# Jorgenlf/Drone-2d-custom-gym-env-for-reinforcement-learning

Measured on AMD Instinct MI355X. Metric: env-steps/sec at 65 536 parallel envs; 1/2/4/8 MI355X scaling, higher is better.
Workload: dtype f64

## Files before the change

### drone-2d-custom-gym-env-for-reinforcement-learning_amd/csrc/d2d_device.h

```cpp
#pragma once
#include <hip/hip_runtime.h>
#include <stdint.h>

#include "../../include/drone2d.h"
#include "d2d_pmath.h"

#pragma clang diagnostic ignored "-Wbitwise-instead-of-logical"

#ifdef D2D_BSTAMP
#define BST_N (1024 * 64 * 8)
__device__ uint64_t d2d_bst[BST_N];
#define BST_ARG , uint64_t* bst = nullptr
#define BST(k, dep)                                                                                      \
    do {                                                                                                 \
        if (bst) {                                                                                       \
            uint64_t bst_v;                                                                              \
            asm volatile("s_memtime %0\n\ts_waitcnt lgkmcnt(0)" : "=s"(bst_v) : "v"(dep));            \
            bst_t[k] = bst_v;                                                                            \
        }                                                                                                \
    } while (0)
#else
#define BST_ARG
#define BST(k, dep) \
    do {       \
// ... 305 lines not shown
constexpr double BR_GOLDEN = 0.3819660112501051;
constexpr double BR_XATOL3 = 1e-6 / 3.0;
constexpr int BT_K_MAX = 48;
template <class S>
__device__ __forceinline__ void brent_init(const S& s, const PathK& K, double px, double py, Brent& B) {
    B.a = 0.0 - 10.0;
    B.b = K.L + 10.0;
    B.fulc = B.a + BR_GOLDEN * (B.b - B.a);
    B.nfc = B.fulc;
    B.xf = B.fulc;
    B.rat = 0.0;
    B.e = 0.0;
    B.ia = u_index(s, B.a);
    B.ib = u_index(s, B.b);
    B.ka = SREC(s, REC_U1, B.ia);
    B.ixf = u_index(s, B.xf);
    B.fx = path_dist_n(s, K, B.xf, B.ixf, px, py, B.kxf);
    B.num = 1;
    B.ffulc = B.fx;
    B.fnfc = B.fx;
}
__device__ __forceinline__ bool brent_open(const Brent& B) {
    const double xm = 0.5 * (B.a + B.b);
    const double tol1 = BR_SQRT_EPS * fabs(B.xf) + BR_XATOL3;
    const double tol2 = 2.0 * tol1;
    return fabs(B.xf - xm) > (tol2 - 0.5 * (B.b - B.a));
}
__device__ __forceinline__ bool brent_active(const Brent& B) { return brent_open(B) & (B.num < 500); }
struct BrCand {
    double x;
    int ix;
};
template <bool KN, class S>
__device__ __forceinline__ int brent_interval(const S& s, const PathK& K, const Brent& B, double x, double ka,
                                              double* kn);
template <bool KN = false, class S>
__device__ __forceinline__ BrCand brent_cand(const S& s, const PathK& K, Brent& B, double* kn = nullptr) {
    const double a = B.a, b = B.b, xf = B.xf, fx = B.fx, nfc = B.nfc, fulc = B.fulc;
    const double ka = S::RM ? B.ka : SREC(s, REC_U1, B.ia);
    const double xm = 0.5 * (a + b);
    const double tol1 = BR_SQRT_EPS * fabs(xf) + BR_XATOL3;
    const double tol2 = 2.0 * tol1;
    const double r = (xf - nfc) * (fx - B.ffulc);
    double q = (xf - fulc) * (fx - B.fnfc);
    double p = (xf - fulc) * q - (xf - nfc) * r;
    q = 2.0 * (q - r);
    p = (q > 0.0) ? -p : p;
    q = fabs(q);
    const bool par = (fabs(B.e) > tol1) & (fabs(p) < fabs(0.5 * q * B.e)) & (p > q * (a - xf)) & (p < q * (b - xf));
    double rat_p = 0.0;
    if (__ballot(par) != 0ull) {
        rat_p = div_normal(p + 0.0, q);
        const double xp = xf + rat_p;
        const double d = xm - xf;
        rat_p = (((xp - a) < tol2) | ((b - xp) < tol2)) ? ((d < 0.0) ? -tol1 : tol1) : rat_p;
    }
    const double e_g = (xf >= xm) ? a - xf : b - xf;
    const double rat_g = BR_GOLDEN * e_g;
    B.e = par ? B.rat : e_g;
    const double rat = par ? rat_p : rat_g;
    B.rat = rat;
    const double mx = max_abs_fin(rat, tol1);
    const double x = xf + copysign(mx, rat);
    return BrCand{x, brent_interval<KN>(s, K, B, x, ka, kn)};
}
template <bool KN, class S>
__device__ __forceinline__ int brent_interval(const S& s, const PathK& K, const Brent& B, double x, double ka,
                                              double* kn) {
    const bool fast = B.ib <= B.ia + 1;
    int ix;
    if (__ballot(!fast) == 0ull) {
        ix = min(B.ia + ((x <= ka) ? 0 : 1), K.nw - 1);
    } else {
        if constexpr (S::RM) {
            int z = 0;
            asm volatile("" : "+v"(z));
            if constexpr (KN) {
                ix = u_index_kn(kn, K.nw, x, z);
            } else {
                ix = u_index_at(s, x, z);
            }
        } else {
            const S* sp = &s;
            asm volatile("" : "+v"(sp));
            ix = u_index(*sp, x);
        }
    }
    return ix;
}
template <class S>
__device__ __forceinline__ bool brent_update(Brent& B, const BrCand& c, double fu, double kx) {
    const double a = B.a, b = B.b, xf = B.xf, fx = B.fx, nfc = B.nfc, fulc = B.fulc;
    const double x = c.x;
    const int ix = c.ix;
    const bool le = fu <= fx;
    const bool c1 = !le & ((fu <= B.fnfc) | (nfc == xf));
    const bool c2 = !le & !c1 & ((fu <= B.ffulc) | (fulc == xf) | (fulc == nfc));
    const bool ge = x >= xf;
    const bool to_a = le == ge;
    const double t = le ? xf : x;
    const int ti = le ? B.ixf : ix;
    B.a = to_a ? t : a;
    B.b = to_a ? b : t;
    B.ia = to_a ? ti : B.ia;
    B.ib = to_a ? B.ib : ti;
    B.ixf = le ? ix : B.ixf;
    if constexpr (S::RM) {
        const double tk = le ? B.kxf : kx;
        B.ka = to_a ? tk : B.ka;
        B.kxf = le ? kx : B.kxf;
    }
    const double nfulc = (le | c1) ? nfc : (c2 ? x : fulc);
    const double nffulc = (le | c1) ? B.fnfc : (c2 ? fu : B.ffulc);
    const double nnfc = le ? xf : (c1 ? x : nfc);
    const double nfnfc = le ? fx : (c1 ? fu : B.fnfc);
    B.fulc = nfulc;
    B.ffulc = nffulc;
    B.nfc = nnfc;
    B.fnfc = nfnfc;
    B.xf = le ? x : xf;
    B.fx = min_fin(fu, fx);
    return le;
}
template <bool KN = false, class S>
__device__ __forceinline__ void brent_step(const S& s, const PathK& K, double px, double py, Brent& B,
                                           double* kn = nullptr BST_ARG) {
#ifdef D2D_BSTAMP
    uint64_t bst_t[5];
#endif
    BST(0, B.xf);
    const bool fast = B.ib <= B.ia + 1;
    const BrCand c = brent_cand<KN>(s, K, B, kn);
    BST(1, c.x);
    BST(2, c.ix);
    double kx;
    const double fu = path_dist_n(s, K, c.x, c.ix, px, py, kx);
    BST(3, fu);
    brent_update<S>(B, c, fu, kx);
#ifdef D2D_BSTAMP
    BST(4, B.fx);
    const uint64_t act = __ballot(1);
    if (bst && (int)(threadIdx.x & 63) == __ffsll((unsigned long long)act) - 1) {
        for (int k = 0; k < 5; ++k) bst[k] = bst_t[k];
        bst[5] = 0;
        bst[6] = (uint64_t)(__ballot(!fast) != 0ull);
        bst[7] = (uint64_t)__popcll(act);
    }
#else
    (void)fast;
#endif
}
template <bool KN = false, class S>
__device__ __forceinline__ void brent_run(const S& s, const PathK& K, double px, double py, Brent& B,
                                          double* kn = nullptr) {
    constexpr int IT_FREE = 500 - (BT_K_MAX + 1);
    for (int it = 0;; ++it) {
        bool act = brent_open(B);
        if (__builtin_expect(it >= IT_FREE, 0)) {
            asm volatile("" ::: "memory");
            act = act & (B.num + it < 500);
        }
        if (!act) break;
#ifdef D2D_BSTAMP
        uint64_t* bst = nullptr;
        if ((threadIdx.x >> 6) == 2 && blockIdx.x < 1024 && it < 64) bst = d2d_bst + ((size_t)blockIdx.x * 64 + it) * 8;
        brent_step<KN>(s, K, px, py, B, kn, bst);
#else
        brent_step<KN>(s, K, px, py, B, kn);
#endif
    }
}
template <bool KN = false, class S>
__device__ __forceinline__ double closest_u(const S& s, double px, double py, int& iu, double* kn = nullptr) {
    static_assert(!KN || S::RM, "staged knots / record cache: global-memory tables only");
    const PathK K = path_k(s);
    if constexpr (KN) {
#pragma unroll
        for (int k = 0; k < D2D_MAX_WPS; ++k) kn[64 * k + (threadIdx.x & 63)] = SUS(s, k);
    }
    Brent B;
    brent_init(s, K, px, py, B);
    brent_run<KN>(s, K, px, py, B, kn);
    iu = B.ixf;
    return B.xf;
}

constexpr int BT_K = BT_K_MAX;
constexpr int BT_HOT = BT_K + 3;
struct BtIt {
    double X, Y;
    double dxn, dxf;
    double e;
    double am, bm;
    double pad;
};
struct BtSnap {
    double a, b, fulc, nfc, xf, rat, e, ka, kxf;
    int32_t num, ia, ib, ixf;
    int32_t j_fulc, j_nfc, j_xf, pad;
};
struct BtHot {
    BtIt it[2][BT_HOT];
};
static_assert(sizeof(BtIt) == 64, "BtIt size");
struct BrTab {
    BtHot hot;
    BtSnap snap[2][BT_K + 1];
    int32_t len[2];
    int32_t pad[2];
};

template <class SC>
__device__ __forceinline__ void brtab_build(const SC& s, int kind, BrTab& T) {
    const PathK K = path_k(s);
    Brent B;
    B.a = 0.0 - 10.0;
    B.b = K.L + 10.0;
    B.fulc = B.a + BR_GOLDEN * (B.b - B.a);
    B.nfc = B.fulc;
    B.xf = B.fulc;
    B.rat = 0.0;
    B.e = 0.0;
    B.ia = u_index(s, B.a);
    B.ib = u_index(s, B.b);
    B.ka = SREC(s, REC_U1, B.ia);
    B.ixf = u_index(s, B.xf);
    B.num = 1;
    B.fx = B.ffulc = B.fnfc = 0.0;
    BtIt& h0 = T.hot.it[kind][0];
    path_eval_n(s, K, B.xf, B.ixf, h0.X, h0.Y, B.kxf);
    h0.dxn = h0.dxf = h0.e = h0.am = h0.bm = h0.pad = 0.0;
    int jf = 0, jn = 0, jx = 0;
    int k = 0;
    for (; k < BT_K && brent_active(B); ++k) {
        BtSnap& S = T.snap[kind][k];
        S = BtSnap{B.a, B.b, B.fulc, B.nfc, B.xf, B.rat, B.e, B.ka, B.kxf, B.num, B.ia, B.ib, B.ixf, jf, jn, jx, 0};
        const double a = B.a, b = B.b, xf = B.xf, nfc = B.nfc, fulc = B.fulc;
        const double xm = 0.5 * (a + b);
        const double tol1 = BR_SQRT_EPS * fabs(xf) + BR_XATOL3;
        BtIt& h = T.hot.it[kind][k + 1];
        h.dxn = xf - nfc;
        h.dxf = xf - fulc;
        h.e = (fabs(B.e) > tol1) ? B.e : 0.0;
        h.am = a - xf;
        h.bm = b - xf;
        h.pad = 0.0;
        const double e_g = (xf >= xm) ? a - xf : b - xf;
        const double rat = BR_GOLDEN * e_g;
        B.e = e_g;
        B.rat = rat;
        const double mx = max_abs_fin(rat, tol1);
        const double x = xf + ((rat < 0.0) ? -mx : mx);
        const int ix = u_index(s, x);
        double kx;
        path_eval_n(s, K, x, ix, h.X, h.Y, kx);
        B.num += 1;
        const bool le = !(kind == 0 && k == 0);
        const bool c1 = !le;
        const bool ge = x >= xf;
        const bool to_a = le == ge;
        const double t = le ? xf : x;
        const int ti = le ? B.ixf : ix;
        const double tk = le ? B.kxf : kx;
        B.a = to_a ? t : a;
        B.b = to_a ? b : t;
        B.ia = to_a ? ti : B.ia;
        B.ka = to_a ? tk : B.ka;
        B.ib = to_a ? B.ib : ti;
        B.ixf = le ? ix : B.ixf;
        B.kxf = le ? kx : B.kxf;
        const int j = k + 1;
        const double nfulc = (le | c1) ? nfc : fulc;
        const int njf = (le | c1) ? jn : jf;
        const double nnfc = le ? xf : (c1 ? x : nfc);
        const int njn = le ? jx : (c1 ? j : jn);
        B.fulc = nfulc;
        B.nfc = nnfc;
        B.xf = le ? x : xf;
        jf = njf;
        jn = njn;
        jx = le ? j : jx;
    }
    T.snap[kind][k] = BtSnap{B.a, B.b, B.fulc, B.nfc, B.xf, B.rat, B.e, B.ka, B.kxf, B.num, B.ia, B.ib, B.ixf,
                             jf, jn, jx, 0};
    T.len[kind] = k;
}

__device__ __forceinline__ double bt_check(const BtIt& h, int k, double px, double py, double ffulc, double fnfc,
                                           double fx, int& dev) {
    const double fu = norm2(h.X - px, h.Y - py);
    const double r = h.dxn * (fx - ffulc);
    double q = h.dxf * (fx - fnfc);
    double p = h.dxf * q - h.dxn * r;
    q = 2.0 * (q - r);
    p = (q > 0.0) ? -p : p;
    q = fabs(q);
    const bool par = (fabs(p) < fabs(0.5 * q * h.e)) & (p > q * h.am) & (p < q * h.bm);
    const bool ok = !par & (fu <= fx);
    dev = min(dev, ok ? BT_HOT : k);
    return fu;
}

template <bool LT>
__device__ __forceinline__ BtIt bt_hot(const BtHot* hot, int kind, int j) {
    if (!LT) return hot->it[kind][j];
    using HL = __attribute__((address_space(3))) const double;
    const HL* q = (const HL*)&hot->it[kind][j];
    return BtIt{q[0], q[1], q[2], q[3], q[4], q[5], q[6], q[7]};
}
template <bool LT>
__device__ __forceinline__ double bt_dist(const BtHot* hot, int kind, int j, double px, double py) {
    const BtIt h = bt_hot<LT>(hot, kind, j);
    return norm2(h.X - px, h.Y - py);
}
struct BtLane {
    int kind, len, dev;
    double fa, fb, fc;
};
template <bool LT>
__device__ __forceinline__ BtLane bt_start(const BrTab& T, const BtHot* hot, double px, double py) {
    const double f0 = bt_dist<LT>(hot, 0, 0, px, py);
    const double f1 = bt_dist<LT>(hot, 0, 1, px, py);
    BtLane L;
    L.kind = (f1 <= f0) ? 1 : 0;
    L.len = T.len[L.kind];
    L.dev = L.len;
    L.fa = f0;
    L.fb = L.kind ? f0 : f1;
    L.fc = L.kind ? f1 : f0;
    return L;
}
template <bool LT>
__device__ __forceinline__ void bt_window(const BtHot* hot, BtLane& L, int k, double px, double py) {
    L.fa = bt_dist<LT>(hot, L.kind, k - 2, px, py);
    L.fb = bt_dist<LT>(hot, L.kind, k - 1, px, py);
    L.fc = bt_dist<LT>(hot, L.kind, k, px, py);
}
template <bool LT>
__device__ __forceinline__ void bt_verify(const BtHot* hot, BtLane& L, int k0, int k1, double px, double py) {
    double fa = L.fa, fb = L.fb, fc = L.fc;
    int dev = L.dev;
    const int kind = L.kind;
    for (int k = k0; __ballot(k < min(dev, k1)) != 0ull; k += 3) {
        BtIt ha{}, hb{}, hc{};
        if (LT || k < min(dev, k1)) {
            ha = bt_hot<LT>(hot, kind, k + 1);
            hb = bt_hot<LT>(hot, kind, k + 2);
            hc = bt_hot<LT>(hot, kind, k + 3);
        }
        const double fd = bt_check(ha, k, px, py, fa, fb, fc, dev);
        const double fe = bt_check(hb, k + 1, px, py, fb, fc, fd, dev);
        const double ff = bt_check(hc, k + 2, px, py, fc, fd, fe, dev);
        fa = fd;
        fb = fe;
        fc = ff;
    }
    L.dev = min(dev, L.len);
    L.fa = fa;
    L.fb = fb;
    L.fc = fc;
}
template <bool LT, class SC>
__device__ __forceinline__ double bt_finish(const SC& s, const BrTab& T, const BtHot* hot, int kind, int dev,
                                            double px, double py, int& iu) {
    const BtSnap& S = T.snap[kind][dev];
    Brent B;
    B.a = S.a;
    B.b = S.b;
    B.fulc = S.fulc;
    B.nfc = S.nfc;
    B.xf = S.xf;
    B.rat = S.rat;
    B.e = S.e;
    B.ka = S.ka;
    B.kxf = S.kxf;
    B.num = S.num;
    B.ia = S.ia;
    B.ib = S.ib;
    B.ixf = S.ixf;
    if (__ballot(brent_active(B)) != 0ull) {
        const PathK K = path_k(s);
        B.ffulc = bt_dist<LT>(hot, kind, S.j_fulc, px, py);
        B.fnfc = bt_dist<LT>(hot, kind, S.j_nfc, px, py);
        B.fx = bt_dist<LT>(hot, kind, S.j_xf, px, py);
        brent_run(s, K, px, py, B);
    }
    iu = B.ixf;
    return B.xf;
}
template <bool LT, class S>
__device__ __forceinline__ double closest_u_tab(const S& s, const BrTab& T, const BtHot* hot, double px,
                                                double py, int& iu) {
    BtLane L = bt_start<LT>(T, hot, px, py);
    bt_verify<LT>(hot, L, 1, BT_K, px, py);
    return bt_finish<LT>(s, T, hot, L.kind, L.dev, px, py, iu);
}
__device__ __forceinline__ int bt_split(const BrTab& T) { return max(4, (T.len[0] + 3) / 2); }
__device__ __forceinline__ int bt_third(const BrTab& T, int p) {
    const int third = (T.len[0] + 2) / 3;
    return p == 0 ? 1 : (p >= 3 ? BT_K : 1 + p * third);
}
template <bool LT>
__device__ __forceinline__ void bt_window_snap(const BrTab& T, const BtHot* hot, BtLane& L, int k0, double px,
                                               double py) {
    const BtSnap& W = T.snap[L.kind][k0];
    L.fa = bt_dist<LT>(hot, L.kind, W.j_fulc, px, py);
    L.fb = bt_dist<LT>(hot, L.kind, W.j_nfc, px, py);
    L.fc = bt_dist<LT>(hot, L.kind, W.j_xf, px, py);
}

struct Body {
    double px, py, a, vx, vy, w;
};

constexpr double M_F = 0.2, M_M = 0.4;

__host__ __device__ constexpr double moment_box(double m, double w, double h) {
    double hw = w / 2.0, hh = h / 2.0;
    double vx[4] = {hw, hw, -hw, -hw}, vy[4] = {-hh, hh, hh, -hh};
    double s1 = 0.0, s2 = 0.0;
    for (int i = 0; i < 4; ++i) {
        double v1x = vx[i] + 0.0, v1y = vy[i] + 0.0;
        double v2x = vx[(i + 1) % 4] + 0.0, v2y = vy[(i + 1) % 4] + 0.0;
        double aa = v2x * v1y - v2y * v1x;
        double bb = (v1x * v1x + v1y * v1y) + (v1x * v2x + v1y * v2y) + (v2x * v2x + v2y * v2y);
        s1 += aa * bb;
        s2 += aa;
    }
    return (m * s1) / (6.0 * s2);
}
constexpr double MI_F = 1.0 / M_F, MI_M = 1.0 / M_M;
constexpr double II_F = 1.0 / moment_box(M_F, 100.0, 10.0);
constexpr double II_M = 1.0 / moment_box(M_M, 20.0, 20.0);

struct Arms {
    double m7c[2], m7s[2];
    double f47c, f47s, f40c, f40s, f33c, f33s;
};
__device__ __forceinline__ void arm(const Arms& A, int k, double& r1x, double& r1y, double& r2x, double& r2y) {
    const int m = k < 3 ? 0 : 1;
    const int q = k % 3;
    r1x = (q == 0) ? -A.m7c[m] : ((q == 1) ? 0.0 : A.m7c[m]);
    r1y = (q == 0) ? -A.m7s[m] : ((q == 1) ? 0.0 : A.m7s[m]);
    const double c = (k == 0 || k == 5) ? A.f47c : ((k == 1 || k == 4) ? A.f40c : A.f33c);
    const double s = (k == 0 || k == 5) ? A.f47s : ((k == 1 || k == 4) ? A.f40s : A.f33s);
    r2x = (k < 3) ? -c : c;
    r2y = (k < 3) ? -s : s;
}

constexpr int ARMS_N = 10;
__device__ __forceinline__ void arms_store(const Arms& A, double* ab, int stride) {
    const double v[ARMS_N] = {A.m7c[0], A.m7c[1], A.m7s[0], A.m7s[1], A.f47c, A.f47s,
                              A.f40c, A.f40s, A.f33c, A.f33s};
#pragma unroll
    for (int q = 0; q < 10; ++q) ab[q * stride] = v[q];
}
__device__ __forceinline__ void arm_lds(const double* ab, int stride, int k, double& r1x, double& r1y, double& r2x,
                                        double& r2y) {
    using LdsD = __attribute__((address_space(3))) double;
    const volatile LdsD* v = (const volatile LdsD*)ab;
    const int m = k < 3 ? 0 : 1;
    const int q = k % 3;
    const double mc = (q == 1) ? 0.0 : v[(0 + m) * stride], ms = (q == 1) ? 0.0 : v[(2 + m) * stride];
    r1x = (q == 0) ? -mc : ((q == 1) ? 0.0 : mc);
    r1y = (q == 0) ? -ms : ((q == 1) ? 0.0 : ms);
    const int f = (k == 0 || k == 5) ? 4 : ((k == 1 || k == 4) ? 6 : 8);
    const double c = v[f * stride], sn = v[(f + 1) * stride];
    r2x = (k < 3) ? -c : c;
    r2y = (k < 3) ? -sn : sn;
}

__device__ __forceinline__ void advance_position(Body& b) {
    b.px = fma(b.vx + 0.0, DT, b.px);
    b.py = fma(b.vy + 0.0, DT, b.py);
    b.a = fma(b.w + 0.0, DT, b.a);
}
template <class S>
__device__ __forceinline__ bool frame_hits(const S& s, const Body& F, double cs, double sn) {
    bool hit = false;
    for (int k = 0; k < s.n_circles; ++k) {
        const double dx = s.cx[k] - F.px, dy = s.cy[k] - F.py;
        {
            const double reach = s.cr[k] + 51.25;
            const bool near = (fabs(dx) < reach) & (fabs(dy) < reach);
            if (__ballot(near) == 0ull) continue;
        }
        const double lx = dx * cs + dy * sn;
        const double ly = -dx * sn + dy * cs;
        const double ex = lx - fmin(fmax(lx, -FRAME_HX), FRAME_HX), ey = ly - fmin(fmax(ly, -FRAME_HY), FRAME_HY);
        const double r = s.cr[k];
        hit |= (ex * ex + ey * ey <= r * r);
    }
    return hit;
}
template <class S>
__device__ __forceinline__ bool phys_positions(const S& s, Body B[3], double fL, double fR, double cs[3],
                                               double sn[3], double& fx, double& fy, double& tq) {
    double c0, s0;
    sincos_d(B[0].a, s0, c0);
    {
        const double tx = B[0].px - (0.0 * c0 - 0.0 * s0), ty = B[0].py - (0.0 * s0 + 0.0 * c0);
        const double cgx = c0 * 0.0 + (-s0) * 0.0 + tx, cgy = s0 * 0.0 + c0 * 0.0 + ty;
        double fwx = c0 * 0.0 + (-s0) * fL, fwy = s0 * 0.0 + c0 * fL;
        double rx = (c0 * -DRONE_R + (-s0) * 0.0 + tx) - cgx, ry = (s0 * -DRONE_R + c0 * 0.0 + ty) - cgy;
        fx = 0.0 + fwx;
        fy = 0.0 + fwy;
        tq = 0.0 + (rx * fwy - ry * fwx);
        fwx = c0 * 0.0 + (-s0) * fR;
        fwy = s0 * 0.0 + c0 * fR;
        rx = (c0 * DRONE_R + (-s0) * 0.0 + tx) - cgx;
        ry = (s0 * DRONE_R + c0 * 0.0 + ty) - cgy;
        fx = fx + fwx;
        fy = fy + fwy;
        tq += rx * fwy - ry * fwx;
    }
#pragma unroll
    for (int i = 0; i < 3; ++i) advance_position(B[i]);
    sincos_d(B[0].a, sn[0], cs[0]);
#pragma unroll
    for (int i = 1; i < 3; ++i) {
        const double d = B[i].a - B[0].a;
        if (!D2D_EXACT_TRIG && fabs(d) < 1e-2) {
            const double d2 = d * d;
            const double sd = d * fma(d2, fma(d2, fma(d2, -1.0 / 5040.0, 1.0 / 120.0), -1.0 / 6.0), 1.0);
            const double cdm1 = d2 * fma(d2, fma(d2, fma(d2, 1.0 / 40320.0, -1.0 / 720.0), 1.0 / 24.0), -0.5);
            sn[i] = fma(sn[0], cdm1, fma(cs[0], sd, sn[0]));
            cs[i] = fma(cs[0], cdm1, fma(-sn[0], sd, cs[0]));
        } else {
            sincos_d(B[i].a, sn[i], cs[i]);
        }
    }
    return frame_hits(s, B[0], cs[0], sn[0]);
}
template <class S>
__device__ __forceinline__ bool frame_advance(const S& s, Body& F) {
    advance_position(F);
    double sn, cs;
    sincos_d(F.a, sn, cs);
    return frame_hits(s, F, cs, sn);
}

__device__ __forceinline__ Arms make_arms(const double cs[3], const double sn[3]) {
    Arms A;
    A.m7c[0] = cs[1] * 7.0; A.m7s[0] = sn[1] * 7.0;
    A.m7c[1] = cs[2] * 7.0; A.m7s[1] = sn[2] * 7.0;
    A.f47c = cs[0] * 47.0; A.f47s = sn[0] * 47.0;
    A.f40c = cs[0] * 40.0; A.f40s = sn[0] * 40.0;
    A.f33c = cs[0] * 33.0; A.f33s = sn[0] * 33.0;
    return A;
}
// ... 385 lines not shown
```

### drone-2d-custom-gym-env-for-reinforcement-learning_amd/csrc/d2d_kernels.h

```cpp
#pragma once
#include <type_traits>

#include "d2d_curriculum.h"
#include "d2d_device.h"
#include "d2d_layout.h"

namespace d2dk {
using namespace d2d;

constexpr int BLOCK = 256;
constexpr int K1_THREADS = 256;
constexpr size_t K1_LDS_BUDGET = 40 * 1024;
constexpr size_t K2_LDS_BUDGET = 64 * 1024;
constexpr int PRIO_W0 = 2, PRIO_W1 = 1, PRIO_W2 = 3, PRIO_W3 = 1, PRIO_W2_POST = 0;

struct StepArgs {
    int n;
    int ns;
    int n_scn;
    double* st;
    int32_t* ist;
    double* acc;
    const void* scn;
    const BrTab* brt;
// ... 40 lines not shown
#define STAMP(k)                                                                                       \
    do {                                                                                               \
        if (a.stamps && (threadIdx.x & 63) == 0)                                                       \
            a.stamps[(size_t)(blockIdx.x * (blockDim.x >> 6) + (threadIdx.x >> 6)) * 8 + (k)] = __builtin_amdgcn_s_memtime(); \
        if (a.stamps && (threadIdx.x & 63) == 0 && (k) == 0)                                           \
            a.stamps[(size_t)(blockIdx.x * (blockDim.x >> 6) + (threadIdx.x >> 6)) * 8 + 7] =                          \
                ((uint64_t)__builtin_amdgcn_s_getreg((3 << 11) | 20) << 32) |                          \
                (uint32_t)__builtin_amdgcn_s_getreg((31 << 11) | 4) | ((uint64_t)(wave & 3) << 36) |   \
                ((uint64_t)(uint32_t)(wg + 1) << 40);                                                  \
    } while (0)
#define D2D_FSTAMP_BASE 65536
#define FSTAMP(k)                                                                                      \
    do {                                                                                               \
        if (a.stamps && (threadIdx.x & 63) == 0)                                                       \
            a.stamps[D2D_FSTAMP_BASE + (size_t)(blockIdx.x * (blockDim.x >> 6) + (threadIdx.x >> 6)) * 8 + (k)] =      \
                __builtin_amdgcn_s_memtime();                                                          \
    } while (0)
#else
#define STAMP(k) \
    do {         \
    } while (0)
#define FSTAMP(k) \
    do {          \
    } while (0)
#endif

__device__ __forceinline__ const BrTab* brtab(const StepArgs& a, int si) { return a.brt ? a.brt + si : nullptr; }
__device__ __forceinline__ size_t rc_entry(const StepArgs& a, int i, uint32_t ep) {
    return (size_t)(ep & 1u) * (size_t)a.ns + (size_t)i;
}

template <bool LDS, int NT, class S>
__device__ __forceinline__ const S* stage_scenarios(const StepArgs& a, S* lds, int first = 0, int count = -1) {
    if (!LDS) return scn_tab<S>(a);
    if (count < 0) count = a.n_scn;
    const int words = count * (int)(sizeof(S) / 8);
    const double* src = reinterpret_cast<const double*>(scn_tab<S>(a) + first);
    double* dst = reinterpret_cast<double*>(lds);
    for (int k = threadIdx.x; k < words; k += NT) dst[k] = src[k];
    return lds - first;
}
template <int NT>
__device__ __forceinline__ const BtHot* stage_hot(const StepArgs& a, BtHot* lds, int first = 0, int count = -1) {
    if (count < 0) count = a.n_scn;
    const int per = (int)(sizeof(BtHot) / 16);
    for (int k = threadIdx.x; k < count * per; k += NT) {
        const double2* src = reinterpret_cast<const double2*>(&a.brt[first + k / per].hot) + (k % per);
        reinterpret_cast<double2*>(lds)[k] = *src;
    }
    return lds - first;
}
template <int NWAVES>
__device__ __forceinline__ void glds_copy(void* lds_dst, const void* gsrc, int bytes) {
    using LP = __attribute__((address_space(3))) void;
    using GP = __attribute__((address_space(1))) void;
    const int wave = __builtin_amdgcn_readfirstlane(threadIdx.x >> 6), lane = threadIdx.x & 63;
    for (int c = wave; c * 1024 < bytes; c += NWAVES) {
        const int off = c * 1024 + lane * 16;
        if (off < bytes)
            __builtin_amdgcn_global_load_lds((GP*)((const char*)gsrc + off), (LP*)((char*)lds_dst + c * 1024), 16, 0, 0);
    }
}

__device__ __forceinline__ size_t fidx(int f, int n, int i) { return (size_t)f * (size_t)n + (size_t)i; }
template <typename T>
__device__ __forceinline__ T& fld(T* base, int f, int n, int i) {
    T* fb = base + (size_t)__builtin_amdgcn_readfirstlane(f) * (size_t)__builtin_amdgcn_readfirstlane(n);
    return fb[i];
}

__device__ __forceinline__ Body load_frame(const StepArgs& a, int i) {
    const int n = a.ns;
    return Body{fld(a.st, 0, n, i), fld(a.st, 1, n, i), fld(a.st, 2, n, i),
                fld(a.st, 3, n, i), fld(a.st, 4, n, i), fld(a.st, 5, n, i)};
}
template <class SC>
__device__ __forceinline__ void spawn_state(const StepArgs& a, const SC& S, int i, uint32_t ep, double sp[7]) {
    double x, y, th;
    spawn_draw(S, a.seed, (uint32_t)a.cfg.env_id_base + (uint32_t)i, ep, x, y, th);
    double sl, cl, sr, cr;
    sincos_d(th + PI, sl, cl);
    sincos_d(th, sr, cr);
    sp[0] = x;
    sp[1] = y;
    sp[2] = th;
    sp[3] = cl * DRONE_R + x;
    sp[4] = sl * DRONE_R + y;
    sp[5] = cr * DRONE_R + x;
    sp[6] = sr * DRONE_R + y;
}

using LdsU32 = __attribute__((address_space(3))) uint32_t;
__device__ __forceinline__ bool flag_seen(const uint32_t& f) {
    return __builtin_amdgcn_readfirstlane(*(const volatile LdsU32*)&f) != 0u;
}
__device__ __forceinline__ int pool_scenario(const StepArgs& a, int j, uint32_t ep) {
    return *a.pool_base + (a.pool_n > 1 ? pool_pick(a.seed, (uint32_t)a.cfg.env_id_base + (uint32_t)j, ep, a.pool_n) : 0);
}
__device__ __forceinline__ int fresh_slot(int j, uint32_t ep) { return 2 * j + (int)(ep & 1u); }
enum { FR_HEAD = 0, FR_TAIL0 = 1, FR_TAIL1 = 2, FR_WORDS = 4 };
__device__ __forceinline__ int next_scenario(const StepArgs& a, int j, uint32_t ep) {
    if (a.cfg.scn_pool == 2) return fresh_slot(j, ep);
    if (a.cfg.scn_pool) return pool_scenario(a, j, ep);
    if (a.n_scn <= 1) return 0;
    return a.env_scn[j];
}

struct K1Shared {
    double cas[6][EPB];
    int scn[EPB];
    uint8_t cause[EPB];
    uint8_t cvalid[EPB];
    uint32_t pflags[EPB];
    uint32_t ep[EPB];
    double sina[EPB];
    uint32_t w0t[EPB], w0fl[EPB];
    uint32_t f_done, f_ca, f_gs, f_rp, f_ver, f_ver1, f_acc, n_tile;
    double pe[2][EPB];
    double acc[D2D_NSTATS][EPB];
    union {
        struct {
            double jb[6 * JB_PER_JOINT][EPB];
            double arms[ARMS_N][EPB];
        } g;
        struct {
            double post[7][EPB];
            alignas(16) float obs[EPB * D2D_OBS_DIM];
        } p;
    } u;
};

__device__ __forceinline__ int lane_fresh() {
    int l;
    asm volatile("v_mbcnt_lo_u32_b32 %0, -1, 0\n\tv_mbcnt_hi_u32_b32 %0, -1, %0" : "=v"(l));
    return l;
}
__device__ __forceinline__ void flag_raise(uint32_t& f) {
    __builtin_amdgcn_fence(__ATOMIC_RELEASE, "workgroup");
    if ((threadIdx.x & 63) == 0) *(volatile LdsU32*)&f = 1u;
}
__device__ __forceinline__ void flag_wait(const uint32_t& f) {
    while (!flag_seen(f)) __builtin_amdgcn_s_sleep(1)  ;
    __builtin_amdgcn_fence(__ATOMIC_ACQUIRE, "workgroup");
}
__device__ __forceinline__ void tile_arrive(uint32_t& c) {
    __builtin_amdgcn_fence(__ATOMIC_RELEASE, "workgroup");
    if ((threadIdx.x & 63) == 0) atomicAdd(&c, 1u);
}
__device__ __forceinline__ void tile_wait(const uint32_t& c, uint32_t n) {
    while (__builtin_amdgcn_readfirstlane(*(const volatile LdsU32*)&c) < n) __builtin_amdgcn_s_sleep(1);
    __builtin_amdgcn_fence(__ATOMIC_ACQUIRE, "workgroup");
}

template <bool LDS, bool LTAB, bool GRP, class S>
__device__ __forceinline__ void k1_stage(const StepArgs& a, S* s_scn, int wg, const S*& scns,
                                         const BtHot*& hots, int& s0) {
    const int ws = (GRP && LDS) ? a.wg_scn[wg] : 0;
    s0 = ws >= 0 ? ws : -ws - 2;
    const int ncopy = (GRP && LDS) ? (ws >= 0 ? 1 : 2) : a.n_scn;
    hots = nullptr;
    if (LDS && (ncopy == 1 || !LTAB)) {
        glds_copy<K1_THREADS / 64>(s_scn, scn_tab<S>(a) + s0, (int)sizeof(S) * ncopy);
        if (LTAB) glds_copy<K1_THREADS / 64>(s_scn + 1, &a.brt[s0].hot, (int)sizeof(BtHot));
        scns = s_scn - s0;
        if (LTAB) hots = reinterpret_cast<const BtHot*>(s_scn + 1) - s0;
    } else {
        scns = stage_scenarios<LDS, K1_THREADS>(a, s_scn, s0, ncopy);
        if (LTAB) hots = stage_hot<K1_THREADS>(a, reinterpret_cast<BtHot*>(s_scn + ncopy), s0, ncopy);
    }
}

extern __shared__ __attribute__((aligned(16))) uint4 d2d_dyn_lds[];
constexpr int K1_KN_BYTES = D2D_MAX_WPS * 64 * 8;
template <bool LDS, bool LTAB, bool GRP, bool S3, class SC>
__device__ __forceinline__ void k1_body(const StepArgs& a, const SC* scns, const BtHot* hots, int s0, K1Shared& sh,
                                        int wg, int role, int qt) {
    const int wave = role;
    const int lane = threadIdx.x & 63;
    const bool gvalid = wg >= 0;
    const int e0 = gvalid ? wg * EPB : 0;
    const int i = e0 + lane;
    const int ie = (GRP && gvalid) ? a.lane_env[i] : i;
    const bool valid = gvalid && (GRP ? ie >= 0 : i < a.n);
    const int n = a.ns;
    const bool auto_reset = a.cfg.auto_reset != 0;
    STAMP(0);
    if (wg == 0 && qt == 0 && a.fill_ctl)
        __hip_atomic_store(&a.fill_ctl[0], __hip_atomic_load(&a.fill_ctl[1], __ATOMIC_RELAXED, __HIP_MEMORY_SCOPE_AGENT),
                           __ATOMIC_RELAXED, __HIP_MEMORY_SCOPE_AGENT);
    if (wg == 0 && qt == 0 && a.clock)
        __hip_atomic_fetch_add(a.clock, (int64_t)1, __ATOMIC_RELAXED, __HIP_MEMORY_SCOPE_AGENT);
    if (wave == 0) sh.scn[lane] = (valid && a.env_scn && a.n_scn > 1) ? a.env_scn[ie] : s0;
    if (S3 && wave == 0) sh.pflags[lane] = 0x7fffffffu;
    Body PF{};
    if (valid && wave != 0) PF = load_frame(a, i);
    if (qt == 0) {
        sh.f_done = 0u;
        sh.f_ca = 0u;
        sh.f_gs = 0u;
        sh.f_rp = 0u;
        sh.f_ver = 0u;
        sh.f_ver1 = 0u;
        sh.f_acc = 0u;
        sh.n_tile = 0u;
    }
    __syncthreads();
    STAMP(1);
    const SC& S = scns[sh.scn[lane]];
    float* const trow = a.tobs ? a.tobs + (size_t)ie * D2D_OBS_DIM : nullptr;
    float* const orow = &sh.u.p.obs[lane * D2D_OBS_DIM];

    Body F0{};
    double path_err = 0.0, tot_rew = 0.0;
    int t = 0, cause = 0;
    uint32_t flags = 0;
    RewardVel RV{};
    double dclose = 0.0, rew_sum = 0.0, rew_pp = 0.0, pdist = 0.0;
    uint32_t plal = 0;
    bool done = false;
    if (wave == 0) {
        __builtin_amdgcn_s_setprio(PRIO_W0);
        double ov[19];
        Body B[3];
        double j[12], cs[3], sn[3], fx = 0.0, fy = 0.0, tq = 0.0;
        if (valid) {
#pragma unroll
            for (int b = 0; b < 3; ++b) {
                B[b].px = fld(a.st, 6 * b + 0, n, i);
                B[b].py = fld(a.st, 6 * b + 1, n, i);
                B[b].a = fld(a.st, 6 * b + 2, n, i);
                B[b].vx = fld(a.st, 6 * b + 3, n, i);
                B[b].vy = fld(a.st, 6 * b + 4, n, i);
                B[b].w = fld(a.st, 6 * b + 5, n, i);
            }
#pragma unroll
            for (int k = 0; k < 12; ++k) j[k] = fld(a.st, D2D_S_J + k, n, i);
            t = fld(a.ist, D2D_I_T, n, i);
            flags = (uint32_t)fld(a.ist, D2D_I_FLAGS, n, i);
            const float2 act = reinterpret_cast<const float2*>(a.act)[ie];
            const float fs = (float)a.cfg.force_scale;
            const float lf = __fmul_rn(__fadd_rn(act.x / 2.0f, 0.5f), fs);
            const float rf = __fmul_rn(__fadd_rn(act.y / 2.0f, 0.5f), fs);
            if (phys_positions(S, B, (double)lf, (double)rf, cs, sn, fx, fy, tq)) flags |= D2D_FLAG_COLLIDED;
            t += 1;
            cause = end_cause(a.cfg, S, B[0], (flags & D2D_FLAG_COLLIDED) != 0, t);
            done = cause != 0;
            const int32_t ep = fld(a.ist, D2D_I_EPISODE, n, i);
            const bool cv = done && auto_reset && a.rc_tag[rc_entry(a, i, (uint32_t)ep)] == ep;
            sh.ep[lane] = (uint32_t)ep;
            sh.cause[lane] = (uint8_t)cause;
            sh.sina[lane] = sn[0];
            sh.cvalid[lane] = cv ? 1u : 0u;
            sh.w0t[lane] = (uint32_t)t;
            sh.w0fl[lane] = flags;
            if (!(done && auto_reset)) {
#pragma unroll
                for (int b = 0; b < 3; ++b) {
                    fld(a.st, 6 * b + 0, n, i) = B[b].px;
                    fld(a.st, 6 * b + 1, n, i) = B[b].py;
                    fld(a.st, 6 * b + 2, n, i) = B[b].a;
                }
            }
        }
        flag_raise(sh.f_done);
        if (valid) {
            const Arms A = make_arms(cs, sn);
            const double pos[6] = {B[0].px, B[0].py, B[1].px, B[1].py, B[2].px, B[2].py};
            double vel[9] = {B[0].vx, B[0].vy, B[0].w, B[1].vx, B[1].vy, B[1].w, B[2].vx, B[2].vy, B[2].w};
            phys_velocities<true>(A, pos, a.damping_dt, fx, fy, tq, vel, j, &sh.u.g.jb[0][lane], EPB,
                                  &sh.u.g.arms[0][lane]);
            asm volatile("" ::: "memory");
            const int ln = lane_fresh(), iw = e0 + ln;
            const uint32_t cw = sh.cause[ln];
            cause = (int)cw;
            done = cw != 0u;
            t = (int)sh.w0t[ln];
            flags = sh.w0fl[ln];
            if (!(done && auto_reset)) {
#pragma unroll
            for (int b = 0; b < 3; ++b) {
                fld(a.st, 6 * b + 3, n, iw) = vel[3 * b + 0];
                fld(a.st, 6 * b + 4, n, iw) = vel[3 * b + 1];
                fld(a.st, 6 * b + 5, n, iw) = vel[3 * b + 2];
            }
#pragma unroll
            for (int k = 0; k < 12; ++k) fld(a.st, D2D_S_J + k, n, iw) = j[k];
            }
            F0 = Body{0.0, 0.0, B[0].a, vel[0], vel[1], vel[2]};
        }
        flag_raise(sh.f_gs);
        STAMP(4);
        const int ln = lane_fresh(), iw = e0 + ln, iew = GRP ? ie : iw;
        const bool vw = gvalid && (GRP ? iew >= 0 : iw < a.n);
        if (vw) {
            float* const orw = &sh.u.p.obs[ln * D2D_OBS_DIM];
            float* const trw = a.tobs ? a.tobs + (size_t)iew * D2D_OBS_DIM : nullptr;
            sensor_vel(F0, sh.sina[ln], cs[0], ov);
            if (!(done && auto_reset)) {
                orw[0] = (float)ov[0];
                orw[1] = (float)ov[1];
                orw[2] = (float)ov[2];
                orw[17] = (float)ov[17];
                orw[18] = (float)ov[18];
            }
            if (done && trw) {
                trw[0] = (float)ov[0];
                trw[1] = (float)ov[1];
                trw[2] = (float)ov[2];
                trw[17] = (float)ov[17];
                trw[18] = (float)ov[18];
            }
        }
        tile_arrive(sh.n_tile);
        flag_wait(sh.f_ca);
        STAMP(5);
        if (vw) {
            CAStatic C;
            C.d = sh.cas[0][ln];
            C.os = sh.cas[1][ln];
            C.oc = sh.cas[2][ln];
            C.lpa = sh.cas[3][ln];
            C.lca = sh.cas[4][ln];
            C.rr = sh.cas[5][ln];
            RV = reward_vel(a.cfg, ov, C);
            dclose = C.d;
        }
        if (!S3) {
            flag_wait(sh.f_acc);
            const int lp = lane_fresh();
            path_err = sh.pe[0][lp];
            tot_rew = sh.pe[1][lp];
        }
        flag_wait(sh.f_rp);
        if (vw) {
            RewardPos RP{};
            RP.aa = sh.u.p.post[4][ln];
            RP.coll = sh.u.p.post[5][ln];
            RP.reach = sh.u.p.post[6][ln];
            RewardPath RQ{};
            RQ.ls = sh.u.p.post[0][ln];
            RQ.lc = sh.u.p.post[1][ln];
            RQ.pa = sh.u.p.post[2][ln];
            if (!GRP) {
                pdist = sh.u.p.post[3][ln];
                plal = sh.pflags[ln];
            }
            const RewardSum Q = reward_sum(a.cfg, RP, RV, RQ);
            rew_sum = Q.reward;
            rew_pp = Q.pp;
        }
    } else if (wave == 1) {
        float row[19];
        bool need = false;
        if (S3) {
            __builtin_amdgcn_s_setprio(PRIO_W2);
            if (valid && a.brt) {
                const BrTab& T = a.brt[sh.scn[lane]];
                const BtHot* hot = LTAB ? hots + sh.scn[lane] : &T.hot;
                Body F = PF;
                advance_position(F);
                BtLane L = bt_start<LTAB>(T, hot, F.px, F.py);
                const int k0 = bt_third(T, 1), k1 = bt_third(T, 2);
                if (k0 < min(k1, L.len)) {
                    if (k0 >= 4) bt_window<LTAB>(hot, L, k0, F.px, F.py);
                else bt_window_snap<LTAB>(T, hot, L, k0, F.px, F.py);
                    bt_verify<LTAB>(hot, L, k0, k1, F.px, F.py);
                }
                atomicMin(&sh.pflags[lane], (uint32_t)L.dev);
            }
            flag_raise(sh.f_ver1);
        }
        __builtin_amdgcn_s_setprio(PRIO_W1);
        if (valid) {
            Body F = PF;
            advance_position(F);
            double so[19];
            sensor_pos(a.cfg, S, F.px, F.py, F.a, so);
            const CAStatic C = ca_static(a.cfg, S, so);
            sh.cas[0][lane] = C.d;
            sh.cas[1][lane] = C.os;
            sh.cas[2][lane] = C.oc;
            sh.cas[3][lane] = C.lpa;
            sh.cas[4][lane] = C.lca;
            sh.cas[5][lane] = C.rr;
#pragma unroll
            for (int k = 0; k < 19; ++k) row[k] = (float)so[k];
        }
        flag_raise(sh.f_ca);
        flag_wait(sh.f_done);
        if (valid) {
            done = sh.cause[lane] != 0u;
            need = done && auto_reset;
            if (done && trow) {
#pragma unroll
                for (int k = 3; k < 17; ++k) trow[k] = row[k];
            }
        }
        if (__ballot(need) != 0ull) {
            if (need) {
                if (sh.cvalid[lane] != 0u) {
                    const float* c = a.rc_obs + rc_entry(a, i, sh.ep[lane]) * D2D_OBS_DIM;
#pragma unroll
                    for (int k = 0; k < 19; ++k) row[k] = c[k];
                } else {
                    const uint32_t ep = sh.ep[lane];
                    const SC& SN = scns[next_scenario(a, ie, ep)];
                    double sp[7], so[19];
                    spawn_state(a, SN, ie, ep, sp);
                    sensor_obs(a.cfg, SN, Body{sp[0], sp[1], sp[2], 0.0, 0.0, 0.0}, so);
#pragma unroll
                    for (int k = 0; k < 19; ++k) row[k] = (float)so[k];
                }
            }
        }
        STAMP(4);
        flag_wait(sh.f_gs);
        STAMP(5);
        if (valid) {
            if (need) {
#pragma unroll
                for (int k = 0; k < 19; ++k) orow[k] = row[k];
            } else {
#pragma unroll
                for (int k = 3; k < 17; ++k) orow[k] = row[k];
            }
        }
        tile_arrive(sh.n_tile);
    } else if (wave == 2) {
        __builtin_amdgcn_s_setprio(PRIO_W2);
        double po[8];
        Body F{};
        if (valid) {
            F = PF;
            advance_position(F);
            uint32_t f = (uint32_t)fld(a.ist, D2D_I_FLAGS, n, i);
            const BrTab* T = brtab(a, sh.scn[lane]);
            if (T) {
                const BtHot* hot = LTAB ? hots + sh.scn[lane] : &T->hot;
                BtLane L = bt_start<LTAB>(*T, hot, F.px, F.py);
                bt_verify<LTAB>(hot, L, 1, !LDS ? BT_K : S3 ? bt_third(*T, 1) : bt_split(*T), F.px, F.py);
                flag_wait(sh.f_ver);
                if (S3) flag_wait(sh.f_ver1);
                L.dev = min(L.dev, (int)sh.pflags[lane]);
                int iu;
                const double u = bt_finish<LTAB>(S, *T, hot, L.kind, L.dev, F.px, F.py, iu);
                path_obs_u(a.cfg, S, F.px, F.py, F.a, u, f, po, iu);
            } else {
                path_obs<LTAB, SC::RM>(a.cfg, S, T, F.px, F.py, F.a, f, po, LTAB ? hots + sh.scn[lane] : nullptr,
                                       SC::RM ? reinterpret_cast<double*>(d2d_dyn_lds) : nullptr);
            }
            sh.pflags[lane] = f & D2D_FLAG_LA_LOCK;
        }
        STAMP(4);
        __builtin_amdgcn_s_setprio(PRIO_W2_POST);
        flag_wait(sh.f_done);
        flag_wait(sh.f_ca);
        RewardPos RP{};
        RewardPath RQ{};
        bool d = false;
        if (valid) {
            const int cause = (int)sh.cause[lane];
            d = cause != 0;
            CAStatic C;
            C.lpa = sh.cas[3][lane];
            RP = reward_pos(a.cfg, F, cause, sh.sina[lane]);
            RQ = reward_path(a.cfg, RP, C, po);
        }
        flag_wait(sh.f_gs);
        if (valid) {
            if (!(d && auto_reset)) {
#pragma unroll
                for (int k = 0; k < 8; ++k) orow[19 + k] = (float)po[k];
            }
            if (d && trow) {
#pragma unroll
                for (int k = 0; k < 8; ++k) trow[19 + k] = (float)po[k];
            }
        }
        if (valid) {
            sh.u.p.post[0][lane] = RQ.ls;
            sh.u.p.post[1][lane] = RQ.lc;
            sh.u.p.post[2][lane] = RQ.pa;
            sh.u.p.post[3][lane] = RQ.dist;
            sh.u.p.post[4][lane] = RP.aa;
            sh.u.p.post[5][lane] = RP.coll;
            sh.u.p.post[6][lane] = RP.reach;
        }
        flag_raise(sh.f_rp);
        tile_arrive(sh.n_tile);
        STAMP(5);
    } else {
        __builtin_amdgcn_s_setprio(PRIO_W2);
        double po[8];
        if (!LDS) {
            sh.pflags[lane] = 0x7fffffffu;
        } else if (valid && a.brt) {
            const BrTab& T = a.brt[sh.scn[lane]];
            const BtHot* hot = LTAB ? hots + sh.scn[lane] : &T.hot;
            Body F = PF;
            advance_position(F);
            BtLane L = bt_start<LTAB>(T, hot, F.px, F.py);
            const int k0 = S3 ? bt_third(T, 2) : bt_split(T);
            if (k0 < L.len) {
                if (k0 >= 4) bt_window<LTAB>(hot, L, k0, F.px, F.py);
                else bt_window_snap<LTAB>(T, hot, L, k0, F.px, F.py);
                bt_verify<LTAB>(hot, L, k0, BT_K, F.px, F.py);
            }
            if (S3) atomicMin(&sh.pflags[lane], (uint32_t)L.dev);
            else sh.pflags[lane] = (uint32_t)L.dev;
        }
        flag_raise(sh.f_ver);
        __builtin_amdgcn_s_setprio(PRIO_W3);
        if (valid) {
            sh.pe[0][lane] = fld(a.st, D2D_S_PATH_ERR, n, i);
            sh.pe[1][lane] = fld(a.st, D2D_S_TOT_REW, n, i);
        }
        flag_wait(sh.f_done);
        const bool cv = valid && sh.cvalid[lane] != 0u;
        if (valid) done = sh.cause[lane] != 0u;
        if (valid && done) {
#pragma unroll
            for (int k = 0; k < D2D_NSTATS; ++k) sh.acc[k][lane] = fld(a.acc, k, n, i);
        }
        flag_raise(sh.f_acc);
        if (valid && done && auto_reset) {
            const uint32_t ep = sh.ep[lane];
            const int nscn = next_scenario(a, ie, ep);
            const SC& SN = scns[nscn];
            double sp[7];
            spawn_state(a, SN, ie, ep, sp);
            uint32_t rfl = 0;
            if (cv) {
                const size_t ce = rc_entry(a, i, ep);
                const float* c = a.rc_obs + ce * D2D_OBS_DIM + 19;
#pragma unroll
                for (int k = 0; k < 8; ++k) po[k] = (double)c[k];
                rfl = (uint32_t)a.rc_rfl[ce];
            } else {
                path_obs(a.cfg, SN, brtab(a, nscn), sp[0], sp[1], sp[2], rfl, po);
            }
            const double th = sp[2];
            const double bodies[18] = {sp[0], sp[1], th, 0.0, 0.0, 0.0, sp[3], sp[4], th, 0.0, 0.0, 0.0,
                                       sp[5], sp[6], th, 0.0, 0.0, 0.0};
#pragma unroll
            for (int f = 0; f < 18; ++f) fld(a.st, f, n, i) = bodies[f];
#pragma unroll
            for (int k = 0; k < 12; ++k) fld(a.st, D2D_S_J + k, n, i) = 0.0;
            fld(a.st, D2D_S_PATH_ERR, n, i) = 0.0;
            fld(a.st, D2D_S_TOT_REW, n, i) = 0.0;
            fld(a.ist, D2D_I_T, n, i) = 0;
            fld(a.ist, D2D_I_FLAGS, n, i) = (int32_t)rfl;
            fld(a.ist, D2D_I_EPISODE, n, i) = (int32_t)(ep + 1u);
            if (a.cfg.scn_pool && a.env_scn) a.env_scn[ie] = nscn;
        }
        if (!LDS && a.fq) {
            const bool need = valid && done && auto_reset;
            const uint64_t m = __ballot(need);
            if (m != 0ull) {
                const int first = __ffsll((unsigned long long)m) - 1;
                uint32_t base = 0;
                if (lane == first) base = atomicAdd(&a.fqc[FR_HEAD], (uint32_t)__popcll(m));
                base = __shfl(base, first);
                const uint32_t pos = base + (uint32_t)__popcll(m & ((1ull << lane) - 1ull));
                if (need) a.fq[pos & a.fq_mask] = fresh_slot(ie, sh.ep[lane] + 1u);
            }
        }
        STAMP(4);
        flag_wait(sh.f_gs);
        STAMP(5);
        if (valid && done && auto_reset) {
#pragma unroll
            for (int k = 0; k < 8; ++k) orow[19 + k] = (float)po[k];
        }
        tile_arrive(sh.n_tile);
    }
    STAMP(2);

    if (wave != 0) {
        tile_wait(sh.n_tile, 4u);
        STAMP(3);
        constexpr int TT = K1_THREADS - 64;
        const int tq = qt - 64;
        if (GRP) {
            for (int k = tq; gvalid && k < EPB * D2D_OBS_DIM; k += TT) {
                const int r = k / D2D_OBS_DIM;
                const int e = a.lane_env[e0 + r];
                if (e >= 0) a.obs[(size_t)e * D2D_OBS_DIM + (k - r * D2D_OBS_DIM)] = sh.u.p.obs[k];
            }
        } else {
            const int rows = gvalid ? max(0, min(EPB, a.n - e0)) : 0;
            const int words = rows * D2D_OBS_DIM;
            float* dst = a.obs + (size_t)e0 * D2D_OBS_DIM;
            int k0 = 0;
            if (rows == EPB && ((uintptr_t)a.obs & 15u) == 0) {
                float4* d4 = reinterpret_cast<float4*>(dst);
                const float4* s4 = reinterpret_cast<const float4*>(sh.u.p.obs);
                for (int k = tq; k < words / 4; k += TT) d4[k] = s4[k];
                k0 = words;
            }
            for (int k = k0 + tq; k < words; k += TT) dst[k] = sh.u.p.obs[k];
        }
    } else {
        if (S3) flag_wait(sh.f_acc);
        STAMP(3);
    }
    const int lne = lane_fresh(), ile = e0 + lne, iee = GRP ? ie : ile;
    const bool vle = gvalid && (GRP ? iee >= 0 : ile < a.n);
    if (wave == 0 && vle) {
        const int lane = lne, i = ile, ie = iee;
        if (S3) {
            path_err = sh.pe[0][lane];
            tot_rew = sh.pe[1][lane];
        }
        flags = (flags & ~D2D_FLAG_LA_LOCK) | (GRP ? sh.pflags[lane] : plal);
        const double reward = rew_sum;
        path_err += GRP ? sh.u.p.post[3][lane] : pdist;
        const double ape_g = GRP ? path_err / (double)t : 0.0;
        tot_rew += reward;
        bool trunc = false, term = done;
        if (a.cfg.timeup_truncates && done && cause == D2D_END_TIMEUP) {
            trunc = true;
            term = false;
        }
        const int io = ie;
        a.rew[io] = (float)reward;
        a.term[io] = (uint8_t)term;
        a.trunc[io] = (uint8_t)trunc;
        if (a.info) {
            float* r = a.info + (size_t)ie * D2D_INFO_DIM;
            r[D2D_INFO_CA] = (float)RV.cal;
            r[D2D_INFO_PA] = (float)sh.u.p.post[2][lane];
            r[D2D_INFO_PP] = (float)rew_pp;
            r[D2D_INFO_COLL] = (float)sh.u.p.post[5][lane];
            r[D2D_INFO_REACH] = (float)sh.u.p.post[6][lane];
            r[D2D_INFO_AA] = (float)sh.u.p.post[4][lane];
            r[D2D_INFO_DCLOSE] = (float)dclose;
            r[D2D_INFO_STEPS] = (float)t;
            r[D2D_INFO_CAUSE] = (float)cause;
            r[D2D_INFO_APE] = done ? (float)(GRP ? ape_g : path_err / (double)t) : 0.0f;
            r[D2D_INFO_TOTREW] = done ? (float)tot_rew : 0.0f;
            r[D2D_INFO_REWARD] = (float)reward;
        }
        if (done) {
            double pacc[D2D_NSTATS];
#pragma unroll
            for (int k = 0; k < D2D_NSTATS; ++k) pacc[k] = sh.acc[k][lane];
            const double ape = GRP ? ape_g : path_err / (double)t;
            const bool c1 = cause & D2D_END_COLLISION, c2 = cause & D2D_END_REACH;
            const bool c4 = cause & D2D_END_TIMEUP, c5 = cause & D2D_END_AA;
            fld(a.acc, D2D_ST_RETURN, n, i) = pacc[D2D_ST_RETURN] + tot_rew;
            fld(a.acc, D2D_ST_EPISODES, n, i) = pacc[D2D_ST_EPISODES] + 1.0;
            fld(a.acc, D2D_ST_SUCCESS, n, i) = pacc[D2D_ST_SUCCESS] + (c2 ? 1.0 : 0.0);
            fld(a.acc, D2D_ST_FAIL, n, i) = pacc[D2D_ST_FAIL] + ((c1 || c4 || c5) ? 1.0 : 0.0);
            fld(a.acc, D2D_ST_COLLISION, n, i) = pacc[D2D_ST_COLLISION] + ((c1 && !c2 && !c4 && !c5) ? 1.0 : 0.0);
            fld(a.acc, D2D_ST_APE, n, i) = pacc[D2D_ST_APE] + ape;
// ... 373 lines not shown
```

Before: 2.492 billion.

## Start Brent refinement speculatively while partner wave finishes table verification

Wave 2 now verifies only the first BT_EARLY table steps, then runs Brent iterations speculatively from that snapshot while wave 3 verifies the remainder. It polls the verify flag and, if the partner finds an earlier deviation, restores from the correct snapshot and restarts. The aim is to overlap wave 2's Brent search with wave 3's verification instead of idling on flag_wait. The cost is possibly wasted speculative iterations, extra LDS polling, and a reduced iteration budget bookkeeping in brent_run.

```diff
diff --git a/drone-2d-custom-gym-env-for-reinforcement-learning_amd/csrc/d2d_device.h b/drone-2d-custom-gym-env-for-reinforcement-learning_amd/csrc/d2d_device.h
--- a/drone-2d-custom-gym-env-for-reinforcement-learning_amd/csrc/d2d_device.h
+++ b/drone-2d-custom-gym-env-for-reinforcement-learning_amd/csrc/d2d_device.h
@@ -481,8 +481,7 @@
 }
 template <bool KN = false, class S>
 __device__ __forceinline__ void brent_run(const S& s, const PathK& K, double px, double py, Brent& B,
-                                          double* kn = nullptr) {
-    constexpr int IT_FREE = 500 - (BT_K_MAX + 1);
+                                          double* kn = nullptr, const int IT_FREE = 500 - (BT_K_MAX + 1)) {
     for (int it = 0;; ++it) {
         bool act = brent_open(B);
         if (__builtin_expect(it >= IT_FREE, 0)) {
@@ -689,11 +688,7 @@
     L.fb = fb;
     L.fc = fc;
 }
-template <bool LT, class SC>
-__device__ __forceinline__ double bt_finish(const SC& s, const BrTab& T, const BtHot* hot, int kind, int dev,
-                                            double px, double py, int& iu) {
-    const BtSnap& S = T.snap[kind][dev];
-    Brent B;
+__device__ __forceinline__ void bt_restore(const BtSnap& S, Brent& B) {
     B.a = S.a;
     B.b = S.b;
     B.fulc = S.fulc;
@@ -707,11 +702,23 @@
     B.ia = S.ia;
     B.ib = S.ib;
     B.ixf = S.ixf;
+}
+template <bool LT>
+__device__ __forceinline__ void bt_restore_f(const BtSnap& S, const BtHot* hot, int kind, double px, double py,
+                                             Brent& B) {
+    B.ffulc = bt_dist<LT>(hot, kind, S.j_fulc, px, py);
+    B.fnfc = bt_dist<LT>(hot, kind, S.j_nfc, px, py);
+    B.fx = bt_dist<LT>(hot, kind, S.j_xf, px, py);
+}
+template <bool LT, class SC>
+__device__ __forceinline__ double bt_finish(const SC& s, const BrTab& T, const BtHot* hot, int kind, int dev,
+                                            double px, double py, int& iu) {
+    const BtSnap& S = T.snap[kind][dev];
+    Brent B;
+    bt_restore(S, B);
     if (__ballot(brent_active(B)) != 0ull) {
         const PathK K = path_k(s);
-        B.ffulc = bt_dist<LT>(hot, kind, S.j_fulc, px, py);
-        B.fnfc = bt_dist<LT>(hot, kind, S.j_nfc, px, py);
-        B.fx = bt_dist<LT>(hot, kind, S.j_xf, px, py);
+        bt_restore_f<LT>(S, hot, kind, px, py, B);
         brent_run(s, K, px, py, B);
     }
     iu = B.ixf;
@@ -725,6 +732,14 @@
     return bt_finish<LT>(s, T, hot, L.kind, L.dev, px, py, iu);
 }
 __device__ __forceinline__ int bt_split(const BrTab& T) { return max(4, (T.len[0] + 3) / 2); }
+#ifndef D2D_BT_EARLY
+#define D2D_BT_EARLY 16
+#endif
+constexpr int BT_EARLY = D2D_BT_EARLY;
+#ifndef D2D_BT_EARLY_GRP
+#define D2D_BT_EARLY_GRP 0
+#endif
+static_assert(BT_EARLY == 0 || (BT_EARLY >= 4 && BT_EARLY % 3 == 1 && BT_EARLY < BT_K), "BT_EARLY");
 __device__ __forceinline__ int bt_third(const BrTab& T, int p) {
     const int third = (T.len[0] + 2) / 3;
     return p == 0 ? 1 : (p >= 3 ? BT_K : 1 + p * third);
diff --git a/drone-2d-custom-gym-env-for-reinforcement-learning_amd/csrc/d2d_kernels.h b/drone-2d-custom-gym-env-for-reinforcement-learning_amd/csrc/d2d_kernels.h
--- a/drone-2d-custom-gym-env-for-reinforcement-learning_amd/csrc/d2d_kernels.h
+++ b/drone-2d-custom-gym-env-for-reinforcement-learning_amd/csrc/d2d_kernels.h
@@ -216,6 +216,40 @@
     __builtin_amdgcn_fence(__ATOMIC_ACQUIRE, "workgroup");
 }
 
+template <bool LT, class SC>
+__device__ __forceinline__ double bt_finish_join(const SC& s, const BrTab& T, const BtHot* hot, const BtLane& L,
+                                                 const uint32_t& fv, const uint32_t& dv, double px, double py,
+                                                 int& iu) {
+    constexpr int IT_JOIN = 200;
+    const PathK K = path_k(s);
+    const bool early = L.dev < L.len;
+    Brent B;
+    bt_restore(T.snap[L.kind][L.dev], B);
+    if (__ballot(early) != 0ull) {
+        if (early) bt_restore_f<LT>(T.snap[L.kind][L.dev], hot, L.kind, px, py, B);
+        uint32_t up = 0u;
+        int it = 0;
+        for (;; ++it) {
+            if (!(early & brent_open(B) & (it < IT_JOIN) & (__builtin_amdgcn_readfirstlane(up) == 0u))) break;
+            up = *(const volatile LdsU32*)&fv;
+            brent_step(s, K, px, py, B);
+        }
+        B.num += it;
+    }
+    flag_wait(fv);
+    const bool late = !early & ((dv < (uint32_t)L.len) | brent_active(B));
+    if (__ballot(late) != 0ull) {
+        if (late) {
+            const BtSnap& S = T.snap[L.kind][min((uint32_t)L.len, dv)];
+            bt_restore(S, B);
+            bt_restore_f<LT>(S, hot, L.kind, px, py, B);
+        }
+    }
+    if (__ballot(brent_active(B)) != 0ull) brent_run(s, K, px, py, B, nullptr, 500 - (BT_K_MAX + 1) - IT_JOIN);
+    iu = B.ixf;
+    return B.xf;
+}
+
 template <bool LDS, bool LTAB, bool GRP, class S>
 __device__ __forceinline__ void k1_stage(const StepArgs& a, S* s_scn, int wg, const S*& scns,
                                          const BtHot*& hots, int& s0) {
@@ -248,6 +282,7 @@
     const bool valid = gvalid && (GRP ? ie >= 0 : i < a.n);
     const int n = a.ns;
     const bool auto_reset = a.cfg.auto_reset != 0;
+    constexpr bool EARLY = LDS && LTAB && !S3 && BT_EARLY > 0 && (!GRP || D2D_BT_EARLY_GRP);
     STAMP(0);
     if (wg == 0 && qt == 0 && a.fill_ctl)
         __hip_atomic_store(&a.fill_ctl[0], __hip_atomic_load(&a.fill_ctl[1], __ATOMIC_RELAXED, __HIP_MEMORY_SCOPE_AGENT),
@@ -502,12 +537,18 @@
             if (T) {
                 const BtHot* hot = LTAB ? hots + sh.scn[lane] : &T->hot;
                 BtLane L = bt_start<LTAB>(*T, hot, F.px, F.py);
-                bt_verify<LTAB>(hot, L, 1, !LDS ? BT_K : S3 ? bt_third(*T, 1) : bt_split(*T), F.px, F.py);
-                flag_wait(sh.f_ver);
-                if (S3) flag_wait(sh.f_ver1);
-                L.dev = min(L.dev, (int)sh.pflags[lane]);
                 int iu;
-                const double u = bt_finish<LTAB>(S, *T, hot, L.kind, L.dev, F.px, F.py, iu);
+                double u;
+                if constexpr (EARLY) {
+                    bt_verify<LTAB>(hot, L, 1, BT_EARLY, F.px, F.py);
+                    u = bt_finish_join<LTAB>(S, *T, hot, L, sh.f_ver, sh.pflags[lane], F.px, F.py, iu);
+                } else {
+                    bt_verify<LTAB>(hot, L, 1, !LDS ? BT_K : S3 ? bt_third(*T, 1) : bt_split(*T), F.px, F.py);
+                    flag_wait(sh.f_ver);
+                    if (S3) flag_wait(sh.f_ver1);
+                    L.dev = min(L.dev, (int)sh.pflags[lane]);
+                    u = bt_finish<LTAB>(S, *T, hot, L.kind, L.dev, F.px, F.py, iu);
+                }
                 path_obs_u(a.cfg, S, F.px, F.py, F.a, u, f, po, iu);
             } else {
                 path_obs<LTAB, SC::RM>(a.cfg, S, T, F.px, F.py, F.a, f, po, LTAB ? hots + sh.scn[lane] : nullptr,
@@ -564,7 +605,7 @@
             Body F = PF;
             advance_position(F);
             BtLane L = bt_start<LTAB>(T, hot, F.px, F.py);
-            const int k0 = S3 ? bt_third(T, 2) : bt_split(T);
+            const int k0 = EARLY ? BT_EARLY : S3 ? bt_third(T, 2) : bt_split(T);
             if (k0 < L.len) {
                 if (k0 >= 4) bt_window<LTAB>(hot, L, k0, F.px, F.py);
                 else bt_window_snap<LTAB>(T, hot, L, k0, F.px, F.py);
```

New measurement: 2.525 billion, median of 6. 1.3% higher.
